# ccaven/tinyslam

Measured on AMD Instinct MI355X. Metric: ORB extract throughput, 1280x720 (frames/sec; Mkeypoints/sec alongside), higher is better.
Workload: dtype f32; 1 GPU; BASELINE.json configs[3]: batch of 256 independent 1280x720 RGBA frames per GPU, device-resident, full ORB (FAST-12 + orientation + blur + BRIEF-256); frames_per_gpu_per_batch=256, width=1280, height=720, hierarchy_depth=2, max_features=8192, content=default, mode=literal, input=rgba, pipeline=default, fp_contract=0, angle_bins=0, batches_in_flight=1, collate=none (1 GPU)

## Files before the change

### include/tinyorb.h

```cpp
#ifndef TINYORB_H
#define TINYORB_H

#include <stddef.h>
#include <stdint.h>

#ifdef __cplusplus
extern "C" {
#endif

#define TINYORB_ABI_VERSION 5

#define ORB_OK 0
#define ORB_EINVAL 1
#define ORB_EHIP 2
#define ORB_ECAPACITY 3
#define ORB_ESTATE 4

#define ORB_MAX_HIERARCHY_DEPTH 10

typedef struct OrbExtent3d {
    uint32_t width;
    uint32_t height;
    uint32_t depth_or_array_layers;
} OrbExtent3d;
// ... 139 lines not shown
    uint32_t reserved[3];
} OrbPairModel;

#define ORB_VERIFY_OK 0u
#define ORB_VERIFY_FEW 1u
#define ORB_VERIFY_DEGENERATE 2u
#define ORB_VERIFY_MINIMAL 3u

int orb_verify_consecutive(OrbProgram *p, uint32_t n_frames, const OrbVerifyParams *params, void *stream);
int orb_verify_read(OrbProgram *p, uint32_t pair, OrbPairModel *model, uint8_t *inlier, size_t n);

void orb_corner_level0_xy(const CornerData *c, float *x0, float *y0);

#define ORB_PLANE_GRAY 0
#define ORB_PLANE_BLUR 1
int orb_debug_read_plane(OrbProgram *p, uint32_t frame, int kind, uint32_t level, uint16_t *dst, size_t n_texels);
int orb_level_size(const OrbProgram *p, uint32_t level, uint32_t *width, uint32_t *height);
int orb_debug_f32_to_f16(OrbProgram *p, const float *src, uint16_t *dst, size_t n);
int orb_debug_angle_code(OrbProgram *p, const float *cy, const float *cx, uint32_t *dst, size_t n);
int orb_debug_rot_table(OrbProgram *p, int16_t *dst, size_t n_entries, uint32_t *codes, uint32_t *pitch);

#define ORB_KERNEL_COUNT 25
int orb_profile_enable(OrbProgram *p, int enable);
int orb_profile_reset(OrbProgram *p);
int orb_profile_get(OrbProgram *p, int id, double *total_ms, uint64_t *launches);
const char *orb_kernel_name(int id);

#define ORB_SYN_GRADIENT 1u
#define ORB_SYN_BLOBS 2u
#define ORB_SYN_WEDGES 4u
// ... 12 lines not shown
```

### tinyslam_amd/csrc/orb_api.hip

```cpp
#include <hip/hip_runtime.h>
#include <chrono>
#include <cmath>

#include <cstdarg>
#include <cstdio>
#include <cstdlib>
#include <cstring>
#include <new>
#include <string>
#include <algorithm>
#include <vector>

#include "../../include/tinyorb.h"
#include "orb_front_launch.h"
#include "orb_kernels_fused.h"
#include "orb_kernels_brief.h"
#include "orb_kernels_intended.h"
#include "orb_kernels_staged.h"
#include "orb_kernels_collate.h"
#include "orb_kernels_match.h"
#include "orb_kernels_verify.h"

using namespace orb;

// ... 110 lines not shown
    uint16_t* d_blur_rowc = nullptr;
    uint32_t blur_qa[kMaxLevels] = {0};
    uint32_t* d_counts = nullptr;
    CornerData* d_corners = nullptr;
    CornerDescriptor* d_desc = nullptr;
    uint32_t* out_counts[2] = {nullptr, nullptr};
    CornerData* out_corners[2] = {nullptr, nullptr};
    CornerDescriptor* out_desc[2] = {nullptr, nullptr};
    CornerData* d_seg = nullptr;
    uint32_t* d_seg_counts = nullptr;
    uint32_t* d_seg_before = nullptr;
    BandGeom bands{};
    RowsGeom rows{};
    BriefTGeom brieft{};
    bool use_brief_t = false;
    uint32_t band_rows_lvl[kMaxLevels] = {0};
    uint32_t ln_threads[kMaxLevels] = {0};
    uint32_t tile_w_lvl[kMaxLevels] = {0};
    uint32_t seg_classes = 1;
    uint32_t* d_pattern = nullptr;
    float* d_cos = nullptr;
    float* d_sin = nullptr;
    uint4* d_rot = nullptr;
    unsigned long long* d_stamps = nullptr;

    uint32_t* h_count = nullptr;
    uint32_t* d_single_done = nullptr;
    hipEvent_t single_done_ev = nullptr;
    uint32_t single_seq = 0;
    CornerData* h_corners = nullptr;
// ... 270 lines not shown
    g.n_classes = n_classes;
    uint32_t rows = 0;
    for (uint32_t m = 0; m < p->pyr.depth; m++) {
        g.flat_end[m] = rg.flat_end[m];
        g.qa[m] = rg.qa[m];
        g.row_base[m] = rows + (uint32_t)kBriefHalo;
        rows += p->pyr.h[m] + 2u * (uint32_t)kBriefHalo + 8u;
    }
    g.rows_padded = rows;
    g.oob = p->oob;
    *out = g;
    if (getenv("TINYORB_BRIEF_ROWS")) return false;
    return rg.n_slots >= 1u && rg.n_slots * n_classes <= kBriefTMaxSlots && rows <= kBriefTMaxRows;
}

int launch_brief(OrbProgram* p, hipStream_t s, uint32_t n, const RowsGeom& rows_geom, const uint16_t* d_blur,
                 const uint16_t* d_blur_rowc, const uint32_t* seg_counts, uint32_t* seg_before, const CornerData* seg,
                 uint32_t* d_counts, CornerData* d_corners, CornerDescriptor* d_desc) {
    const uint32_t cap = p->cfg.max_features;
    const BriefTables tab{p->d_pattern, p->d_cos, p->d_sin, p->d_rot};
    const bool use_t = p->use_brief_t;
    {
        LaunchScope ls(p, s, KID_PREFIX);
        hipLaunchKernelGGL(k_slot_prefix, dim3(n), dim3(64), 0, s, seg_counts, seg_before, d_counts, rows_geom.n_slots,
                           rows_geom.seg_cap, use_t ? p->brieft.n_classes : 1u);
    }
    if (use_t) {
        const BriefTGeom& tg = p->brieft;
        const dim3 grid(n, (cap + (uint32_t)kBriefNfChunk - 1u) / (uint32_t)kBriefNfChunk);
        {
            LaunchScope ls(p, s, KID_BRIEF_T);
#define BRIEF_T_LAUNCH(ROT_)                                                                                                         \
    hipLaunchKernelGGL((k_brief_t<kBriefTWaves, ROT_>), dim3(n, (cap + kBriefTThreads - 1u) / kBriefTThreads), dim3(kBriefTThreads), \
                       brieft_lds_bytes(tg), s, d_blur_rowc, p->pyr, tg, seg_counts, seg_before, seg, d_corners, cap, d_desc, tab)
            switch (rot_form(p->opt.fp_contract)) {
                case 1: BRIEF_T_LAUNCH(1); break;
                case 2: BRIEF_T_LAUNCH(2); break;
                default: BRIEF_T_LAUNCH(0); break;
            }
#undef BRIEF_T_LAUNCH
        }
        LaunchScope ls(p, s, KID_BRIEF_NF);
        if (p->oob != kOobZero)
            hipLaunchKernelGGL(k_brief_nf<true>, grid, dim3(256), 0, s, d_blur, d_blur_rowc, p->pyr, tg, seg_counts, seg_before, d_corners,
                               cap, d_desc, tab);
        else
            hipLaunchKernelGGL(k_brief_nf<false>, grid, dim3(256), 0, s, d_blur, d_blur_rowc, p->pyr, tg, seg_counts, seg_before, d_corners,
                               cap, d_desc, tab);
    } else {
        LaunchScope ls(p, s, KID_BRIEF_ROWS);
        RowsGeom rg = rows_geom;
        rg.oob = p->oob;
        rg.fp = p->opt.fp_contract;
        rg.split = 1u;
        while (rg.split < 16u && rg.n_slots * n * rg.split < 2048u) rg.split *= 2u;
        hipLaunchKernelGGL(k_brief_rows, dim3(rg.n_slots * rg.split, n), dim3(256), 0, s, d_blur, d_blur_rowc, p->pyr, rg,
                           seg_counts, seg_before, seg, d_corners, cap, d_desc, tab);
    }
    return ORB_OK;
}

int run_fused_range(OrbProgram* p, const uint8_t* frames_all, uint32_t f0, uint32_t n, hipStream_t s, bool with_brief = true,
                    uint32_t first_level = 0) {
    const Pyramid& pyr = p->pyr;
// ... 40 lines not shown
        if (!g.tiled && sizeof(BlurCol) * (size_t)g.n_var > 8u * (size_t)g.ts)
            return fail(p, ORB_EINVAL, "internal: blur column table of level %u does not fit", lvl);
        uint32_t lds = front_lds_bytes(g);
        lds += (uint32_t)p->env.lds_pad;
        if (lds > p->max_lds) return fail(p, ORB_EINVAL, "level %u needs %u bytes of LDS", lvl, lds);
        const dim3 grid(g.n_bands * (g.tiled ? g.n_ct : 1u) * n);
        FrontLaunch L{frames, p->frame_bytes, d_gray, d_blur, d_blur_rowc, pyr, g, p->threshold, d_seg_counts, d_seg, s_lvl, grid.x, lds,
                      p->band_rows_lvl[lvl], p->ln_threads[lvl], p->input_y8,
                      lvl == 0 && ((pyr.w[0] & 3u) || g.store_grey), p->oob != kOobZero, false};
        {
            LaunchScope ls(p, s_lvl, lvl == 0 ? KID_FUSED_L0 : KID_FUSED_LN);
            const hipError_t e = kFrontLaunch[front_form(p->opt.fp_contract, lvl == 0 && !p->input_y8)](L);
            if (e != hipSuccess) return fail(p, ORB_EHIP, "k_front (level %u) failed to launch: %s", lvl, hipGetErrorString(e));
        }
    }
    if (with_brief) launch_brief(p, s, n, p->rows, d_blur, d_blur_rowc, d_seg_counts, d_seg_before, d_seg, d_counts, d_corners, d_desc);
    HIP_TRY(p, hipGetLastError());
    return ORB_OK;
}

int run_fused(OrbProgram* p, const uint8_t* frames, uint32_t n, hipStream_t s) {
    if (int rc = run_fused_range(p, frames, 0, n, s)) return rc;
    p->planes_valid = true;
    return ORB_OK;
}

uint32_t itile_width(uint32_t w) {
    const uint32_t w8 = (w + 7u) & ~7u;
    return w8 < (uint32_t)kITileW ? w8 : (uint32_t)kITileW;
}

// ... 146 lines not shown
            fg.slot_base = band_base;
            fg.n_slots = p->xband_slots;
            fg.seg_cap = 1u;
            fg.n_classes = 1u;
            fg.stamps = nullptr;
            band_base += fg.n_bands;
            const uint32_t lds = front_lds_bytes(fg);
            if (lds > p->max_lds) return fail(p, ORB_EINVAL, "level %u needs %u bytes of LDS", lvl, lds);
            LaunchScope ls(p, s, KID_FUSED_LN);
            const FrontLaunch L{frames, p->frame_bytes, p->d_gray, p->d_blur, p->d_blur_rowc, pyr, fg, p->threshold, p->d_xband_counts, p->d_iseg, s,
                                fg.n_bands * n, lds, (uint32_t)kFrontRows, (uint32_t)kFrontThreadsLN, false, false, false, true};
            const hipError_t e = kFrontLaunch[0](L);
            if (e != hipSuccess) return fail(p, ORB_EHIP, "k_front (blur of level %u) failed to launch: %s", lvl, hipGetErrorString(e));
        }
    }
    launch_brief(p, s, n, p->xrows, p->d_blur, p->d_blur_rowc, p->d_iseg_counts, p->d_iseg_before, p->d_iseg, p->d_counts,
                 p->d_corners, p->d_desc);
    HIP_TRY(p, hipGetLastError());
    p->planes_valid = true;
    return ORB_OK;
}

int launch_compact(OrbProgram* p, uint32_t n, uint32_t* counts, uint64_t* offsets, CornerData* corners, CornerDescriptor* desc,
                   size_t capacity, void* stream, hipStream_t* used);

int run_pipeline(OrbProgram* p, const uint8_t* frames, uint32_t n, hipStream_t s) {
    if (p->fused_i) return run_fused_i(p, frames, n, s);
    if (p->fused_x) return run_fused_x(p, frames, n, s);
    return p->fused ? run_fused(p, frames, n, s) : run_staged(p, frames, n, s);
}

// ... 339 lines not shown
    p->d_desc = p->out_desc[0];
    if (p->fused) {
        CREATE_TRY(hipMalloc(&p->d_blur_rowc, B * p->pyr.row_stride * sizeof(uint16_t)));
        CREATE_TRY(hipMemset(p->d_blur_rowc, 0, B * p->pyr.row_stride * sizeof(uint16_t)));
        const size_t lists = (size_t)p->bands.n_slots * p->seg_classes;
        CREATE_TRY(hipMalloc(&p->d_seg, B * lists * (size_t)p->bands.seg_cap * sizeof(CornerData)));
        CREATE_TRY(hipMalloc(&p->d_seg_counts, B * lists * sizeof(uint32_t)));
        CREATE_TRY(hipMemset(p->d_seg_counts, 0, B * lists * sizeof(uint32_t)));
        CREATE_TRY(hipMalloc(&p->d_seg_before, B * lists * sizeof(uint32_t)));
    }
    if (p->fused_x) {
        CREATE_TRY(hipMalloc(&p->d_blur_rowc, B * p->pyr.row_stride * sizeof(uint16_t)));
        CREATE_TRY(hipMemset(p->d_blur_rowc, 0, B * p->pyr.row_stride * sizeof(uint16_t)));
        CREATE_TRY(hipMalloc(&p->d_xband_counts, B * (size_t)p->xband_slots * sizeof(uint32_t)));
    }
    if (p->fused_i || p->fused_x) {
        const size_t n_seg = B * (size_t)p->itiles.n_slots;
        CREATE_TRY(hipMalloc(&p->d_iseg, n_seg * p->itiles.seg_cap * sizeof(CornerData)));
        CREATE_TRY(hipMalloc(&p->d_iseg_scores, n_seg * p->itiles.seg_cap * sizeof(float)));
        CREATE_TRY(hipMalloc(&p->d_iseg_counts, n_seg * sizeof(uint32_t)));
        CREATE_TRY(hipMemset(p->d_iseg_counts, 0, n_seg * sizeof(uint32_t)));
        CREATE_TRY(hipMalloc(&p->d_iseg_before, n_seg * sizeof(uint32_t)));
        CREATE_TRY(hipMalloc(&p->d_thr_key, B * sizeof(unsigned long long)));
    } else if (p->opt.flags & (ORB_FLAG_NMS | ORB_FLAG_INTENDED)) {
        uint32_t off = 0, width = W, height = H;
        for (uint32_t m = 0; m < p->pyr.depth; m++) {
            const uint32_t gw = ((width + 7u) / 8u) * 8u, gh = ((height + 7u) / 8u) * 8u;
            p->score_layout.off[m] = off;
            p->score_layout.pitch[m] = gw + 2u;
            off += (gw + 2u) * (gh + 2u);
// ... 66 lines not shown
    (void)hipFree(p->d_input);
    (void)hipFree(p->d_input_alt);
    for (hipEvent_t ev : p->in_uploaded)
        if (ev) (void)hipEventDestroy(ev);
    (void)hipFree(p->d_gray);
    (void)hipFree(p->d_blur);
    (void)hipFree(p->d_blur_rowc);
    for (int set = 0; set < 2; set++) {
        (void)hipFree(p->out_counts[set]);
        (void)hipFree(p->out_corners[set]);
        (void)hipFree(p->out_desc[set]);
    }
    (void)hipFree(p->d_seg);
    (void)hipFree(p->d_seg_counts);
    (void)hipFree(p->d_seg_before);
    (void)hipFree(p->d_score_planes);
    (void)hipFree(p->d_prov_counts);
    (void)hipFree(p->d_prov);
    (void)hipFree(p->d_prov_scores);
    (void)hipFree(p->d_matches);
    (void)hipFree(p->d_xband_counts);
    (void)hipFree(p->d_iseg);
    (void)hipFree(p->d_iseg_scores);
    (void)hipFree(p->d_iseg_counts);
    (void)hipFree(p->d_iseg_before);
    (void)hipFree(p->d_thr_key);
    (void)hipFree(p->d_prov2_counts);
    (void)hipFree(p->d_prov2);
    (void)hipFree(p->d_prov2_scores);
    (void)hipFree(p->d_pattern);
// ... 767 lines not shown
    if (counts) *counts = p->d_counts;
    if (corners) *corners = p->d_corners;
    if (descriptors) *descriptors = p->d_desc;
    return ORB_OK;
}

int orb_level_size(const OrbProgram* p, uint32_t level, uint32_t* width, uint32_t* height) {
    if (!p || level >= p->pyr.depth) return ORB_EINVAL;
    if (width) *width = p->pyr.w[level];
    if (height) *height = p->pyr.h[level];
    return ORB_OK;
}

int orb_debug_read_plane(OrbProgram* p, uint32_t frame, int kind, uint32_t level, uint16_t* dst, size_t n_texels) {
    if (!p) return ORB_EINVAL;
    if (!dst || level >= p->pyr.depth || frame >= p->last_batch || (kind != ORB_PLANE_GRAY && kind != ORB_PLANE_BLUR))
        return fail(p, ORB_EINVAL, "debug_read_plane: bad arguments");
    if (!p->planes_valid || ((p->fused || (p->fused_i && !p->igrey_stored)) && kind == ORB_PLANE_GRAY && level == 0))
        return fail(p, ORB_ESTATE, "plane not materialised by the last call");
    const size_t texels = (size_t)p->pyr.w[level] * p->pyr.h[level];
    if (n_texels != texels) return fail(p, ORB_EINVAL, "debug_read_plane: expected %zu texels", texels);
    if (int rc = orb_batch_sync(p)) return rc;
    const uint16_t* base = (kind == ORB_PLANE_GRAY ? p->d_gray : p->d_blur) + (size_t)frame * p->pyr.stride + p->pyr.off[level];
    HIP_TRY(p, hipMemcpy(dst, base, texels * sizeof(uint16_t), hipMemcpyDeviceToHost));
    if ((p->fused || p->fused_x) && kind == ORB_PLANE_BLUR && p->blur_qa[level] > 0) {
        const uint32_t w = p->pyr.w[level], h = p->pyr.h[level], qa = p->blur_qa[level];
        std::vector<uint16_t> rowc(h);
        HIP_TRY(p, hipMemcpy(rowc.data(), p->d_blur_rowc + (size_t)frame * p->pyr.row_stride + p->pyr.row_off[level],
                             h * sizeof(uint16_t), hipMemcpyDeviceToHost));
        for (uint32_t y = 0; y < h; y++)
// ... 133 lines not shown
```

### tinyslam_amd/csrc/orb_kernels_brief.h

```cpp
#pragma once
#include "orb_kernels_fused.h"

namespace orb {

constexpr int kBriefTThreads = 256;
constexpr int kBriefTWaves = 6;
constexpr uint32_t kBriefTMaxSlots = 8192;
constexpr uint32_t kBriefTMaxRows = 12288;

struct BriefTGeom {
    uint32_t n_slots, seg_cap;
    uint32_t n_classes;
    uint32_t flat_end[kMaxLevels];
    uint32_t qa[kMaxLevels];
    uint32_t row_base[kMaxLevels];
    uint32_t rows_padded;
    uint32_t oob;
};

__host__ __device__ inline uint32_t brieft_lds_bytes(const BriefTGeom& g) {
    return (g.n_slots * g.n_classes + 1u) * 4u + ((g.rows_padded + 1u) & ~1u) * 2u;
}

__device__ __forceinline__ constexpr int pat_ax(int j) { return ORB_BRIEF_PATTERN[4 * j + 0]; }
// ... 20 lines not shown
}

__device__ __forceinline__ void brief_t_stage_rows(uint16_t* rows, const uint16_t* __restrict__ src, const Pyramid& pyr,
                                                   const BriefTGeom& bg, uint32_t tid, uint32_t n_threads = kBriefTThreads) {
    uint32_t m = 0;
    for (uint32_t i = tid; i < bg.rows_padded; i += n_threads) {
        while (m + 1u < pyr.depth && i + (uint32_t)kBriefHalo >= bg.row_base[m + 1u]) m++;
        const uint32_t y = i - bg.row_base[m];
        uint16_t v = 0;
        if (y < pyr.h[m]) v = src[pyr.row_off[m] + y];
        else if (bg.oob != kOobZero) v = src[pyr.row_off[m] + (uint32_t)oob_index((int)y, (int)pyr.h[m], bg.oob)];
        rows[i] = v;
    }
}

template <int CHUNK = kBriefTThreads, bool STAGED = false, int ROT = 0>
__device__ __forceinline__ void brief_t_body(uint8_t* lds_raw, uint32_t frame, uint32_t chunk, const uint16_t* __restrict__ blur_rowc,
                                             const Pyramid& pyr, const BriefTGeom& bg, const uint32_t* __restrict__ seg_counts,
                                             const uint32_t* __restrict__ seg_before, const CornerData* __restrict__ segments,
                                             CornerData* __restrict__ corners, uint32_t cap,
                                             CornerDescriptor* __restrict__ descriptors, const BriefTables& tab,
                                             CornerData* __restrict__ host_corners = nullptr,
                                             CornerDescriptor* __restrict__ host_descriptors = nullptr) {
    const uint32_t n_ent = bg.n_slots * bg.n_classes;
    uint32_t* const before = reinterpret_cast<uint32_t*>(lds_raw);
    uint16_t* const rows = reinterpret_cast<uint16_t*>(before + n_ent + 1u);
    __shared__ uint32_t lv[kMaxLevels][2];

    const uint32_t tid = threadIdx.x;
    const size_t sbase = (size_t)frame * n_ent;
    uint32_t stored_total;
    if (STAGED) {
        if (tid < pyr.depth) lv[tid][0] = bg.flat_end[tid], lv[tid][1] = bg.row_base[tid];
        __syncthreads();
        stored_total = before[n_ent];
    } else {
        stored_total = seg_before[sbase + n_ent - 1u] + min(seg_counts[sbase + n_ent - 1u], bg.seg_cap);
    }
    const uint32_t n_frame = min(stored_total, cap);
    const uint32_t k0 = chunk * (uint32_t)CHUNK;
    if (k0 >= n_frame) return;

    if (!STAGED) {
        for (uint32_t s = tid; s < n_ent; s += kBriefTThreads) before[s] = seg_before[sbase + s];
        if (tid == 0) before[n_ent] = stored_total;
        if (tid < pyr.depth) lv[tid][0] = bg.flat_end[tid], lv[tid][1] = bg.row_base[tid];
        brief_t_stage_rows(rows, blur_rowc + (size_t)frame * pyr.row_stride, pyr, bg, tid);
        __syncthreads();
    }

    const uint32_t k = k0 + tid;
    if (tid >= (uint32_t)CHUNK || k >= n_frame) return;
    uint32_t lo = 0, hi = n_ent;
    while (hi - lo > 1u) {
        const uint32_t mid = (lo + hi) >> 1;
        if (before[mid] <= k)
            lo = mid;
        else
            hi = mid;
    }
    const uint32_t cls = lo >= bg.n_slots ? 1u : 0u, slot = lo - cls * bg.n_slots;
    const uint4 rec = *reinterpret_cast<const uint4*>(
        &segments[(((size_t)frame * bg.n_slots + slot) * bg.n_classes + cls) * bg.seg_cap + (k - before[lo])]);
    *reinterpret_cast<uint4*>(&corners[(size_t)frame * cap + k]) = rec;
    if (host_corners) store_host_16(&host_corners[k], rec);
    const uint32_t lvl = min(rec.w, pyr.depth - 1u);
    if (!(rec.x >= (uint32_t)kBriefHalo && rec.x < lv[lvl][0])) return;

    uint32_t d[8];
    uint4* const o = reinterpret_cast<uint4*>(descriptors + (size_t)frame * cap + k);
    if (bg.n_classes == 2u && k0 + (tid & ~63u) + 64u <= before[bg.n_slots]) {
        const uint16_t* base0 = rows + lv[lvl][1] + rec.y - kBriefHalo;
#pragma unroll
        for (int wd = 0; wd < 8; wd++) {
            uint32_t acc = 0;
#pragma unroll
            for (int i = 31; i >= 0; i--) {
                const int j = wd * 32 + i;
                acc = push_gt(acc, base0[pat_ay(j) + kBriefHalo], base0[pat_by(j) + kBriefHalo]);
            }
            d[wd] = acc;
        }
// ... 31 lines not shown
            acc = push_gt(acc, base[(int)ray], base[(int)rby]);
        }
        d[wd] = acc;
    }
    o[0] = make_uint4(d[0], d[1], d[2], d[3]);
    o[1] = make_uint4(d[4], d[5], d[6], d[7]);
    if (host_descriptors) {
        store_host_16(reinterpret_cast<uint4*>(host_descriptors + k), make_uint4(d[0], d[1], d[2], d[3]));
        store_host_16(reinterpret_cast<uint4*>(host_descriptors + k) + 1, make_uint4(d[4], d[5], d[6], d[7]));
    }
}

template <int kWavesPerSimd, int ROT = 0>
__global__ __launch_bounds__(kBriefTThreads, kWavesPerSimd) void k_brief_t(const uint16_t* __restrict__ blur_rowc, Pyramid pyr, BriefTGeom bg,
                                                                const uint32_t* __restrict__ seg_counts,
                                                                const uint32_t* __restrict__ seg_before,
                                                                const CornerData* __restrict__ segments,
                                                                CornerData* __restrict__ corners, uint32_t cap,
                                                                CornerDescriptor* __restrict__ descriptors, BriefTables tab) {
    extern __shared__ __attribute__((aligned(16))) uint8_t lds_raw[];
    brief_t_body<kBriefTThreads, false, ROT>(lds_raw, blockIdx.x, blockIdx.y, blur_rowc, pyr, bg, seg_counts, seg_before, segments, corners, cap, descriptors, tab);
}

constexpr int kNfPatchCols = 48, kNfPatchRows = 2 * kBriefHalo + 1;
constexpr int kNfPatchHalfs = kNfPatchRows * kNfPatchCols;

__global__ __launch_bounds__(64) void k_rot_table(const uint32_t* __restrict__ pattern, const float* __restrict__ cos_tab,
                                                  const float* __restrict__ sin_tab, int pitch, int intended, uint4* __restrict__ out,
                                                  uint32_t fp = 0u, uint32_t angle_bins = 0u) {
    const uint32_t code = angle_bins ? (blockIdx.x * 6284u + 3142u) / angle_bins : blockIdx.x, lane = threadIdx.x;
    const float ct = cos_tab[code], st = sin_tab[code], nst = -st;
    uint32_t w[4];
#pragma unroll
    for (int e = 0; e < 4; e++) {
        const uint32_t pk = pattern[64u * (uint32_t)e + lane];
        const float pax = (float)(int8_t)(pk & 255u), pay = (float)(int8_t)((pk >> 8) & 255u);
// ... 2 lines not shown
        if (intended) {
            const float a0 = ct * pax, a1 = nst * pay, a2 = st * pax, a3 = ct * pay;
            const float b0 = ct * pbx, b1 = nst * pby, b2 = st * pbx, b3 = ct * pby;
            rax = a0 + a1, ray = a2 + a3, rbx = b0 + b1, rby = b2 + b3;
        } else {
            rotate_fp(ct, st, nst, pax, pay, rot_form(fp), &rax, &ray);
            rotate_fp(ct, st, nst, pbx, pby, rot_form(fp), &rbx, &rby);
        }
        const int oa = 2 * ((int)ray * pitch + (int)rax), ob = 2 * ((int)rby * pitch + (int)rbx);
        w[e] = ((uint32_t)oa & 0xffffu) | ((uint32_t)ob << 16);
    }
    out[(size_t)blockIdx.x * 64u + lane] = make_uint4(w[0], w[1], w[2], w[3]);
}
__device__ __forceinline__ int rot_a(uint32_t w) { return (int)(int16_t)(w & 0xffffu); }
__device__ __forceinline__ int rot_b(uint32_t w) { return (int)w >> 16; }

template <int CHUNK = 256, int NW = 4, bool OOB = false>
__device__ __forceinline__ void brief_nf_body(uint32_t frame, uint32_t chunk, uint32_t n_known, const uint16_t* __restrict__ blur,
                                              const uint16_t* __restrict__ blur_rowc, const Pyramid& pyr, const BriefTGeom& bg,
                                              const uint32_t* __restrict__ seg_counts, const uint32_t* __restrict__ seg_before,
                                              const CornerData* __restrict__ corners, uint32_t cap,
                                              CornerDescriptor* __restrict__ descriptors, const BriefTables& tab,
                                              CornerDescriptor* __restrict__ host_descriptors = nullptr) {
    static_assert(CHUNK <= 256 && NW >= 4, "the scan runs on the first four waves");
    __shared__ __attribute__((aligned(16))) uint16_t patches[NW][kNfPatchHalfs];
    __shared__ uint4 recs[256];
    __shared__ uint16_t list[256];
    __shared__ uint32_t wave_n[4];
    __shared__ uint32_t lv[kMaxLevels][6];
    const uint32_t tid = threadIdx.x, lane = tid & 63u, wave = tid >> 6;
// ... 127 lines not shown
                    vb = plane[(size_t)(uint32_t)(__mul24(yb, w) + xb)];
                bal[e] = __ballot(va > vb);
            }
        }
        if (lane < 8u) {
            const uint64_t src = lane < 2u ? bal[0] : (lane < 4u ? bal[1] : (lane < 6u ? bal[2] : bal[3]));
            out_desc[(size_t)idx * 8u + lane] = (uint32_t)(src >> ((lane & 1u) * 32u));
            if (host_descriptors) store_host_u32(reinterpret_cast<uint32_t*>(host_descriptors + k0) + (size_t)idx * 8u + lane, (uint32_t)(src >> ((lane & 1u) * 32u)));
        }
    }
}

constexpr int kBriefNfChunk = 64;
template <bool OOB = false>
__global__ __launch_bounds__(256) void k_brief_nf(const uint16_t* __restrict__ blur, const uint16_t* __restrict__ blur_rowc,
                                                  Pyramid pyr, BriefTGeom bg, const uint32_t* __restrict__ seg_counts,
                                                  const uint32_t* __restrict__ seg_before,
                                                  const CornerData* __restrict__ corners, uint32_t cap,
                                                  CornerDescriptor* __restrict__ descriptors, BriefTables tab) {
    brief_nf_body<kBriefNfChunk, 4, OOB>(blockIdx.x, blockIdx.y, ~0u, blur, blur_rowc, pyr, bg, seg_counts, seg_before, corners, cap, descriptors, tab);
}

constexpr int kBriefOneChunk = 64;
constexpr int kSingleCountWords = 32, kSingleDoneWord = 16;
constexpr int kBriefOneThreads = 512;
template <int ROT = 0>
__global__ __launch_bounds__(kBriefOneThreads) void k_brief_one(const uint16_t* __restrict__ blur, const uint16_t* __restrict__ blur_rowc, Pyramid pyr,
                                                   BriefTGeom bg, const uint32_t* __restrict__ seg_counts,
                                                   uint32_t* __restrict__ seg_before, const CornerData* __restrict__ segments,
                                                   uint32_t* __restrict__ counts, CornerData* __restrict__ corners, uint32_t cap,
                                                   CornerDescriptor* __restrict__ descriptors, BriefTables tab,
                                                   uint32_t* __restrict__ host_count, CornerData* __restrict__ host_corners,
                                                   CornerDescriptor* __restrict__ host_descriptors, uint32_t* __restrict__ done_count,
                                                   uint32_t seq) {
    extern __shared__ __attribute__((aligned(16))) uint8_t lds_raw[];
// ... 24 lines not shown
            const uint32_t stored = min(raw, bg.seg_cap);
            const uint32_t incl = wave_inclusive_sum(stored);
            if (e < n_ent) before[e] = carry + incl - stored;
            carry += (uint32_t)__builtin_amdgcn_readlane((int)incl, 63);
            total += (uint32_t)__builtin_amdgcn_readlane((int)wave_inclusive_sum(raw), 63);
        }
        if (tid == 0u) {
            before[n_ent] = carry;
            if (chunk == 0u) {
                counts[0] = total;
                store_host_u32(host_count, total);
            }
        }
    }
    BRIEF_ONE_STAMP();
    brief_t_body<kBriefOneChunk, true, ROT>(lds_raw, 0u, chunk, blur_rowc, pyr, bg, seg_counts, seg_before, segments, corners, cap,
                                       descriptors, tab, host_corners, host_descriptors);
    __syncthreads();
    BRIEF_ONE_STAMP();
    const uint32_t n_stored = before[n_ent];
    brief_nf_body<kBriefOneChunk, kBriefOneThreads / 64>(0u, chunk, n_stored, blur, blur_rowc, pyr, bg, seg_counts, seg_before, corners, cap, descriptors, tab,
                                  host_descriptors);
    BRIEF_ONE_STAMP();
    __builtin_amdgcn_fence(__ATOMIC_RELEASE, "workgroup");
    __builtin_amdgcn_s_waitcnt(0);
    __syncthreads();
    BRIEF_ONE_STAMP();
#ifdef TINYORB_STAMPS
    if (tid == 0u && (chunk == 0u || chunk == 24u))
        for (int i = 0; i < 5; i++) host_count[(chunk ? 6 : 1) + i] = (uint32_t)(st[i + 1] - st[i]);
#endif
// ... 13 lines not shown
```

### tinyslam_amd/orb.py

```python
import ctypes
import importlib.util
import os
from dataclasses import dataclass, field

import numpy as np

_PKG = os.path.dirname(os.path.abspath(__file__))
LIB_PATH = os.environ.get("TINYORB_LIB") or os.path.join(os.path.dirname(os.path.abspath(__file__)), "libtinyorb.so")

ORB_OK, ORB_EINVAL, ORB_EHIP, ORB_ECAPACITY, ORB_ESTATE = 0, 1, 2, 3, 4
ORB_PLANE_GRAY, ORB_PLANE_BLUR = 0, 1
ORB_KERNEL_COUNT = 25
ORB_FLAG_STAGED = 1
ORB_FLAG_DOUBLE_OUTPUT = 2
ORB_FLAG_NMS = 4
ORB_FLAG_INTENDED = 8
ORB_FLAG_INPUT_Y8 = 16
ORB_FLAG_SINGLE_BLOCKING_WAIT = 32
ORB_OOB_ZERO, ORB_OOB_CLAMP, ORB_OOB_UMIN = 0, 1, 2
OOB_POLICIES = {"zero": ORB_OOB_ZERO, "clamp": ORB_OOB_CLAMP, "umin": ORB_OOB_UMIN}
ORB_FP_CONTRACT_LUMINANCE, ORB_FP_CONTRACT_BLUR, ORB_FP_CONTRACT_ROTATION, ORB_FP_CONTRACT_ALL, ORB_FP_LAST_TERM_FIRST = 1, 2, 4, 7, 8
TRANSPORT_RECORD_WORDS = 10
SYN_GRADIENT, SYN_BLOBS, SYN_WEDGES, SYN_NOISE = 1, 2, 4, 8
SYN_ALL = 15

CORNER_DTYPE = np.dtype([("x", "<u4"), ("y", "<u4"), ("angle", "<u4"), ("octave", "<u4")])
# ... 606 lines not shown
```

Baseline: 478,200 frames/s.

## Fold slot prefix into k_brief_t and emit compacted non-flat keypoint lists

Removes the separate k_slot_prefix launch on the k_brief_t path: each brief_t block recomputes the per-frame segment prefix sum in LDS and chunk 0 writes the frame total. brief_t also ballots and compacts keypoints that fall outside the flat fast path into a per-wave list, so k_brief_nf processes only those entries (one wave per keypoint) instead of rescanning all corners. This saves a launch and the nf kernel's scan work, at the cost of redundant prefix work in every block plus extra list memory and writes.

```diff
diff --git a/include/tinyorb.h b/include/tinyorb.h
--- a/include/tinyorb.h
+++ b/include/tinyorb.h
@@ -177,6 +177,7 @@
 
 #define ORB_PLANE_GRAY 0
 #define ORB_PLANE_BLUR 1
+#define ORB_PLANE_NF_COUNT 2
 int orb_debug_read_plane(OrbProgram *p, uint32_t frame, int kind, uint32_t level, uint16_t *dst, size_t n_texels);
 int orb_level_size(const OrbProgram *p, uint32_t level, uint32_t *width, uint32_t *height);
 int orb_debug_f32_to_f16(OrbProgram *p, const float *src, uint16_t *dst, size_t n);
diff --git a/tinyslam_amd/csrc/orb_api.hip b/tinyslam_amd/csrc/orb_api.hip
--- a/tinyslam_amd/csrc/orb_api.hip
+++ b/tinyslam_amd/csrc/orb_api.hip
@@ -148,6 +148,9 @@
     RowsGeom rows{};
     BriefTGeom brieft{};
     bool use_brief_t = false;
+    uint4* d_nf_list = nullptr;
+    uint32_t* d_nf_count = nullptr;
+    uint32_t nf_chunks = 0;
     uint32_t band_rows_lvl[kMaxLevels] = {0};
     uint32_t ln_threads[kMaxLevels] = {0};
     uint32_t tile_w_lvl[kMaxLevels] = {0};
@@ -448,25 +451,20 @@
     return rg.n_slots >= 1u && rg.n_slots * n_classes <= kBriefTMaxSlots && rows <= kBriefTMaxRows;
 }
 
-int launch_brief(OrbProgram* p, hipStream_t s, uint32_t n, const RowsGeom& rows_geom, const uint16_t* d_blur,
+int launch_brief(OrbProgram* p, hipStream_t s, uint32_t f0, uint32_t n, const RowsGeom& rows_geom, const uint16_t* d_blur,
                  const uint16_t* d_blur_rowc, const uint32_t* seg_counts, uint32_t* seg_before, const CornerData* seg,
                  uint32_t* d_counts, CornerData* d_corners, CornerDescriptor* d_desc) {
     const uint32_t cap = p->cfg.max_features;
     const BriefTables tab{p->d_pattern, p->d_cos, p->d_sin, p->d_rot};
-    const bool use_t = p->use_brief_t;
-    {
-        LaunchScope ls(p, s, KID_PREFIX);
-        hipLaunchKernelGGL(k_slot_prefix, dim3(n), dim3(64), 0, s, seg_counts, seg_before, d_counts, rows_geom.n_slots,
-                           rows_geom.seg_cap, use_t ? p->brieft.n_classes : 1u);
-    }
-    if (use_t) {
+    if (p->use_brief_t) {
         const BriefTGeom& tg = p->brieft;
+        const NfList nf{p->d_nf_list + (size_t)f0 * p->nf_chunks * 64u, p->d_nf_count + (size_t)f0 * p->nf_chunks, p->nf_chunks};
         const dim3 grid(n, (cap + (uint32_t)kBriefNfChunk - 1u) / (uint32_t)kBriefNfChunk);
         {
             LaunchScope ls(p, s, KID_BRIEF_T);
 #define BRIEF_T_LAUNCH(ROT_)                                                                                                         \
     hipLaunchKernelGGL((k_brief_t<kBriefTWaves, ROT_>), dim3(n, (cap + kBriefTThreads - 1u) / kBriefTThreads), dim3(kBriefTThreads), \
-                       brieft_lds_bytes(tg), s, d_blur_rowc, p->pyr, tg, seg_counts, seg_before, seg, d_corners, cap, d_desc, tab)
+                       brieft_lds_bytes(tg), s, d_blur_rowc, p->pyr, tg, seg_counts, seg, d_counts, d_corners, cap, d_desc, tab, nf)
             switch (rot_form(p->opt.fp_contract)) {
                 case 1: BRIEF_T_LAUNCH(1); break;
                 case 2: BRIEF_T_LAUNCH(2); break;
@@ -476,12 +474,15 @@
         }
         LaunchScope ls(p, s, KID_BRIEF_NF);
         if (p->oob != kOobZero)
-            hipLaunchKernelGGL(k_brief_nf<true>, grid, dim3(256), 0, s, d_blur, d_blur_rowc, p->pyr, tg, seg_counts, seg_before, d_corners,
-                               cap, d_desc, tab);
+            hipLaunchKernelGGL(k_brief_nf<true>, grid, dim3(256), 0, s, d_blur, d_blur_rowc, p->pyr, tg, nf, cap, d_desc, tab);
         else
-            hipLaunchKernelGGL(k_brief_nf<false>, grid, dim3(256), 0, s, d_blur, d_blur_rowc, p->pyr, tg, seg_counts, seg_before, d_corners,
-                               cap, d_desc, tab);
+            hipLaunchKernelGGL(k_brief_nf<false>, grid, dim3(256), 0, s, d_blur, d_blur_rowc, p->pyr, tg, nf, cap, d_desc, tab);
     } else {
+        {
+            LaunchScope ls(p, s, KID_PREFIX);
+            hipLaunchKernelGGL(k_slot_prefix, dim3(n), dim3(64), 0, s, seg_counts, seg_before, d_counts, rows_geom.n_slots,
+                               rows_geom.seg_cap, 1u);
+        }
         LaunchScope ls(p, s, KID_BRIEF_ROWS);
         RowsGeom rg = rows_geom;
         rg.oob = p->oob;
@@ -552,7 +553,7 @@
             if (e != hipSuccess) return fail(p, ORB_EHIP, "k_front (level %u) failed to launch: %s", lvl, hipGetErrorString(e));
         }
     }
-    if (with_brief) launch_brief(p, s, n, p->rows, d_blur, d_blur_rowc, d_seg_counts, d_seg_before, d_seg, d_counts, d_corners, d_desc);
+    if (with_brief) launch_brief(p, s, f0, n, p->rows, d_blur, d_blur_rowc, d_seg_counts, d_seg_before, d_seg, d_counts, d_corners, d_desc);
     HIP_TRY(p, hipGetLastError());
     return ORB_OK;
 }
@@ -729,7 +730,7 @@
             if (e != hipSuccess) return fail(p, ORB_EHIP, "k_front (blur of level %u) failed to launch: %s", lvl, hipGetErrorString(e));
         }
     }
-    launch_brief(p, s, n, p->xrows, p->d_blur, p->d_blur_rowc, p->d_iseg_counts, p->d_iseg_before, p->d_iseg, p->d_counts,
+    launch_brief(p, s, 0, n, p->xrows, p->d_blur, p->d_blur_rowc, p->d_iseg_counts, p->d_iseg_before, p->d_iseg, p->d_counts,
                  p->d_corners, p->d_desc);
     HIP_TRY(p, hipGetLastError());
     p->planes_valid = true;
@@ -1099,6 +1100,12 @@
         CREATE_TRY(hipMemset(p->d_blur_rowc, 0, B * p->pyr.row_stride * sizeof(uint16_t)));
         CREATE_TRY(hipMalloc(&p->d_xband_counts, B * (size_t)p->xband_slots * sizeof(uint32_t)));
     }
+    if (p->use_brief_t) {
+        p->nf_chunks = 4u * (uint32_t)((cap + kBriefTThreads - 1u) / kBriefTThreads);
+        CREATE_TRY(hipMalloc(&p->d_nf_list, B * p->nf_chunks * 64u * sizeof(uint4)));
+        CREATE_TRY(hipMalloc(&p->d_nf_count, B * p->nf_chunks * sizeof(uint32_t)));
+        CREATE_TRY(hipMemset(p->d_nf_count, 0, B * p->nf_chunks * sizeof(uint32_t)));
+    }
     if (p->fused_i || p->fused_x) {
         const size_t n_seg = B * (size_t)p->itiles.n_slots;
         CREATE_TRY(hipMalloc(&p->d_iseg, n_seg * p->itiles.seg_cap * sizeof(CornerData)));
@@ -1195,6 +1202,8 @@
     (void)hipFree(p->d_seg);
     (void)hipFree(p->d_seg_counts);
     (void)hipFree(p->d_seg_before);
+    (void)hipFree(p->d_nf_list);
+    (void)hipFree(p->d_nf_count);
     (void)hipFree(p->d_score_planes);
     (void)hipFree(p->d_prov_counts);
     (void)hipFree(p->d_prov);
@@ -1992,6 +2001,15 @@
 
 int orb_debug_read_plane(OrbProgram* p, uint32_t frame, int kind, uint32_t level, uint16_t* dst, size_t n_texels) {
     if (!p) return ORB_EINVAL;
+    if (kind == ORB_PLANE_NF_COUNT && dst && level == 0 && frame < p->last_batch) {
+        if (!p->use_brief_t || p->single_valid) return fail(p, ORB_ESTATE, "the last call was no batch of the k_brief_t path");
+        if (n_texels != p->nf_chunks) return fail(p, ORB_EINVAL, "debug_read_plane: expected %u chunk counts", p->nf_chunks);
+        if (int rc = orb_batch_sync(p)) return rc;
+        std::vector<uint32_t> c(p->nf_chunks);
+        HIP_TRY(p, hipMemcpy(c.data(), p->d_nf_count + (size_t)frame * p->nf_chunks, c.size() * sizeof(uint32_t), hipMemcpyDeviceToHost));
+        for (size_t i = 0; i < c.size(); i++) dst[i] = (uint16_t)c[i];
+        return ORB_OK;
+    }
     if (!dst || level >= p->pyr.depth || frame >= p->last_batch || (kind != ORB_PLANE_GRAY && kind != ORB_PLANE_BLUR))
         return fail(p, ORB_EINVAL, "debug_read_plane: bad arguments");
     if (!p->planes_valid || ((p->fused || (p->fused_i && !p->igrey_stored)) && kind == ORB_PLANE_GRAY && level == 0))
diff --git a/tinyslam_amd/csrc/orb_kernels_brief.h b/tinyslam_amd/csrc/orb_kernels_brief.h
--- a/tinyslam_amd/csrc/orb_kernels_brief.h
+++ b/tinyslam_amd/csrc/orb_kernels_brief.h
@@ -58,35 +58,64 @@
     }
 }
 
+struct NfList {
+    uint4* entries;
+    uint32_t* count;
+    uint32_t chunks;
+};
+
 template <int CHUNK = kBriefTThreads, bool STAGED = false, int ROT = 0>
 __device__ __forceinline__ void brief_t_body(uint8_t* lds_raw, uint32_t frame, uint32_t chunk, const uint16_t* __restrict__ blur_rowc,
                                              const Pyramid& pyr, const BriefTGeom& bg, const uint32_t* __restrict__ seg_counts,
-                                             const uint32_t* __restrict__ seg_before, const CornerData* __restrict__ segments,
+                                             const CornerData* __restrict__ segments,
                                              CornerData* __restrict__ corners, uint32_t cap,
                                              CornerDescriptor* __restrict__ descriptors, const BriefTables& tab,
                                              CornerData* __restrict__ host_corners = nullptr,
-                                             CornerDescriptor* __restrict__ host_descriptors = nullptr) {
+                                             CornerDescriptor* __restrict__ host_descriptors = nullptr,
+                                             uint32_t* __restrict__ counts = nullptr, NfList nf = {}) {
     const uint32_t n_ent = bg.n_slots * bg.n_classes;
     uint32_t* const before = reinterpret_cast<uint32_t*>(lds_raw);
     uint16_t* const rows = reinterpret_cast<uint16_t*>(before + n_ent + 1u);
     __shared__ uint32_t lv[kMaxLevels][2];
 
-    const uint32_t tid = threadIdx.x;
-    const size_t sbase = (size_t)frame * n_ent;
+    const uint32_t tid = threadIdx.x, lane = tid & 63u, wave = tid >> 6;
     uint32_t stored_total;
     if (STAGED) {
         if (tid < pyr.depth) lv[tid][0] = bg.flat_end[tid], lv[tid][1] = bg.row_base[tid];
         __syncthreads();
         stored_total = before[n_ent];
     } else {
-        stored_total = seg_before[sbase + n_ent - 1u] + min(seg_counts[sbase + n_ent - 1u], bg.seg_cap);
+        const uint32_t* sc = seg_counts + (size_t)frame * n_ent;
+        uint32_t carry = 0, total = 0;
+        for (uint32_t e0 = 0; e0 < n_ent; e0 += 256u) {
+            uint32_t raw[4];
+#pragma unroll
+            for (int q = 0; q < 4; q++) {
+                const uint32_t e = e0 + 64u * (uint32_t)q + lane;
+                const uint32_t cls = e >= bg.n_slots ? 1u : 0u, sl = e - cls * bg.n_slots;
+                raw[q] = e < n_ent ? sc[sl * bg.n_classes + cls] : 0u;
+            }
+#pragma unroll
+            for (int q = 0; q < 4; q++) {
+                const uint32_t e = e0 + 64u * (uint32_t)q + lane;
+                const uint32_t stored = min(raw[q], bg.seg_cap);
+                const uint32_t incl = wave_inclusive_sum(stored);
+                if ((uint32_t)q == wave && e < n_ent) before[e] = carry + incl - stored;
+                carry += (uint32_t)__builtin_amdgcn_readlane((int)incl, 63);
+                if (chunk == 0u) total += (uint32_t)__builtin_amdgcn_readlane((int)wave_inclusive_sum(raw[q]), 63);
+            }
+        }
+        if (chunk == 0u && tid == 0u) counts[frame] = total;
+        stored_total = carry;
     }
     const uint32_t n_frame = min(stored_total, cap);
     const uint32_t k0 = chunk * (uint32_t)CHUNK;
-    if (k0 >= n_frame) return;
+    if (k0 >= n_frame) {
+        if (!STAGED && tid < 4u) nf.count[(size_t)frame * nf.chunks + 4u * chunk + tid] = 0u;
+        return;
+    }
 
     if (!STAGED) {
-        for (uint32_t s = tid; s < n_ent; s += kBriefTThreads) before[s] = seg_before[sbase + s];
         if (tid == 0) before[n_ent] = stored_total;
         if (tid < pyr.depth) lv[tid][0] = bg.flat_end[tid], lv[tid][1] = bg.row_base[tid];
         brief_t_stage_rows(rows, blur_rowc + (size_t)frame * pyr.row_stride, pyr, bg, tid);
@@ -94,22 +123,34 @@
     }
 
     const uint32_t k = k0 + tid;
-    if (tid >= (uint32_t)CHUNK || k >= n_frame) return;
+    if (STAGED && (tid >= (uint32_t)CHUNK || k >= n_frame)) return;
+    const bool valid = STAGED || k < n_frame;
+    const uint32_t kq = STAGED ? k : min(k, n_frame - 1u);
     uint32_t lo = 0, hi = n_ent;
     while (hi - lo > 1u) {
         const uint32_t mid = (lo + hi) >> 1;
-        if (before[mid] <= k)
+        if (before[mid] <= kq)
             lo = mid;
         else
             hi = mid;
     }
     const uint32_t cls = lo >= bg.n_slots ? 1u : 0u, slot = lo - cls * bg.n_slots;
     const uint4 rec = *reinterpret_cast<const uint4*>(
-        &segments[(((size_t)frame * bg.n_slots + slot) * bg.n_classes + cls) * bg.seg_cap + (k - before[lo])]);
-    *reinterpret_cast<uint4*>(&corners[(size_t)frame * cap + k]) = rec;
+        &segments[(((size_t)frame * bg.n_slots + slot) * bg.n_classes + cls) * bg.seg_cap + (kq - before[lo])]);
+    if (valid) *reinterpret_cast<uint4*>(&corners[(size_t)frame * cap + k]) = rec;
     if (host_corners) store_host_16(&host_corners[k], rec);
     const uint32_t lvl = min(rec.w, pyr.depth - 1u);
-    if (!(rec.x >= (uint32_t)kBriefHalo && rec.x < lv[lvl][0])) return;
+    const bool flat = rec.x >= (uint32_t)kBriefHalo && rec.x < lv[lvl][0];
+    if (!STAGED) {
+        const uint64_t m = __ballot(valid && !flat);
+        const size_t q = (size_t)frame * nf.chunks + 4u * chunk + wave;
+        if (valid && !flat)
+            nf.entries[q * 64u + (uint32_t)__popcll(m & ((1ull << lane) - 1ull))] =
+                make_uint4(rec.x, rec.y, min(rec.z, (uint32_t)(ORB_ANGLE_STEPS - 1)), lvl | (lane << 8));
+        if (lane == 0u) nf.count[q] = (uint32_t)__popcll(m);
+        if (!valid) return;
+    }
+    if (!flat) return;
 
     uint32_t d[8];
     uint4* const o = reinterpret_cast<uint4*>(descriptors + (size_t)frame * cap + k);
@@ -171,12 +212,12 @@
 template <int kWavesPerSimd, int ROT = 0>
 __global__ __launch_bounds__(kBriefTThreads, kWavesPerSimd) void k_brief_t(const uint16_t* __restrict__ blur_rowc, Pyramid pyr, BriefTGeom bg,
                                                                 const uint32_t* __restrict__ seg_counts,
-                                                                const uint32_t* __restrict__ seg_before,
-                                                                const CornerData* __restrict__ segments,
+                                                                const CornerData* __restrict__ segments, uint32_t* __restrict__ counts,
                                                                 CornerData* __restrict__ corners, uint32_t cap,
-                                                                CornerDescriptor* __restrict__ descriptors, BriefTables tab) {
+                                                                CornerDescriptor* __restrict__ descriptors, BriefTables tab, NfList nf) {
     extern __shared__ __attribute__((aligned(16))) uint8_t lds_raw[];
-    brief_t_body<kBriefTThreads, false, ROT>(lds_raw, blockIdx.x, blockIdx.y, blur_rowc, pyr, bg, seg_counts, seg_before, segments, corners, cap, descriptors, tab);
+    brief_t_body<kBriefTThreads, false, ROT>(lds_raw, blockIdx.x, blockIdx.y, blur_rowc, pyr, bg, seg_counts, segments, corners, cap, descriptors,
+                                             tab, nullptr, nullptr, counts, nf);
 }
 
 constexpr int kNfPatchCols = 48, kNfPatchRows = 2 * kBriefHalo + 1;
@@ -209,6 +250,102 @@
 }
 __device__ __forceinline__ int rot_a(uint32_t w) { return (int)(int16_t)(w & 0xffffu); }
 __device__ __forceinline__ int rot_b(uint32_t w) { return (int)w >> 16; }
+
+template <bool OOB>
+__device__ __forceinline__ void brief_nf_key(uint32_t lane, uint16_t* patch, const uint4& r, int w, int h, int qa,
+                                             const uint16_t* __restrict__ rowc, const uint16_t* __restrict__ plane, const BriefTGeom& bg,
+                                             const BriefTables& tab, uint32_t* out_desc, uint32_t idx) {
+    const uint4 tt = tab.rot[(size_t)min(r.z, (uint32_t)(ORB_ANGLE_STEPS - 1)) * 64u + lane];
+    const uint32_t tw[4] = {tt.x, tt.y, tt.z, tt.w};
+    uint64_t bal[4];
+    if ((w & 1) == 0) {
+        const int c0 = ((int)r.x - kBriefHalo) & ~7;
+        constexpr int kPiecesPerRow = kNfPatchCols / 8, kPieces = kNfPatchRows * kPiecesPerRow;
+        constexpr int kRounds = (kPieces + 63) / 64;
+        uint4 tv[kRounds];
+        uint32_t rcv[kRounds];
+        int kind[kRounds], where[kRounds];
+#pragma unroll
+        for (int rr = 0; rr < kRounds; rr++) {
+            const int p = (int)lane + 64 * rr;
+            const int pr = (int)(((float)p + 0.5f) * (1.0f / (float)kPiecesPerRow));
+            const int pc = p - pr * kPiecesPerRow;
+            const int gy0 = (int)r.y - kBriefHalo + pr, cx = c0 + 8 * pc;
+            const int gy = OOB ? oob_index(gy0, h, bg.oob) : gy0;
+            const bool in = p < kPieces && gy >= 0 && gy < h && cx >= 0 && cx < w;
+            kind[rr] = !in ? 0 : (cx < qa ? 1 : (cx + 8 <= w ? 2 : 3));
+            where[rr] = p < kPieces ? pr * kNfPatchCols + 8 * pc : -1;
+            rcv[rr] = rowc[min(max(gy, 0), h - 1)];
+            if (OOB && p < kPieces && !(cx >= 0 && cx < w)) {
+                const int xm = oob_index(cx, w, bg.oob);
+                if (xm >= qa) rcv[rr] = plane[(size_t)(uint32_t)(__mul24(gy, w) + xm)];
+                kind[rr] = 1;
+            }
+            tv[rr] = *reinterpret_cast<const uint4*>(plane + (kind[rr] == 2 ? (size_t)(uint32_t)(__mul24(gy, w) + cx) : (size_t)0));
+        }
+#pragma unroll
+        for (int rr = 0; rr < kRounds; rr++) {
+            uint4 v = make_uint4(0u, 0u, 0u, 0u);
+            if (kind[rr] == 1) {
+                const uint32_t c2 = rcv[rr] | (rcv[rr] << 16);
+                v = make_uint4(c2, c2, c2, c2);
+            } else if (kind[rr] == 2) {
+                v = tv[rr];
+            } else if (kind[rr] == 3) {
+                const int p = (int)lane + 64 * rr;
+                const int pr = (int)(((float)p + 0.5f) * (1.0f / (float)kPiecesPerRow));
+                const int gy0 = (int)r.y - kBriefHalo + pr, cx = c0 + 8 * (p - pr * kPiecesPerRow);
+                const int gy = OOB ? oob_index(gy0, h, bg.oob) : gy0;
+                const uint16_t* src = plane + (size_t)(uint32_t)(__mul24(gy, w) + cx);
+                uint32_t t[8];
+#pragma unroll
+                for (int q = 0; q < 8; q++) t[q] = cx + q < w ? (uint32_t)src[q] : (OOB ? (uint32_t)src[w - 1 - cx] : 0u);
+                v = make_uint4(t[0] | (t[1] << 16), t[2] | (t[3] << 16), t[4] | (t[5] << 16), t[6] | (t[7] << 16));
+            }
+            if (where[rr] >= 0) *reinterpret_cast<uint4*>(&patch[where[rr]]) = v;
+        }
+        __builtin_amdgcn_fence(__ATOMIC_RELEASE, "wavefront");
+        __builtin_amdgcn_wave_barrier();
+        const int xo = (int)r.x - c0;
+        const uint8_t* const centre = reinterpret_cast<const uint8_t*>(patch + kBriefHalo * kNfPatchCols + xo);
+#pragma unroll
+        for (int e = 0; e < 4; e++) {
+            const uint32_t va = *reinterpret_cast<const uint16_t*>(centre + rot_a(tw[e]));
+            const uint32_t vb = *reinterpret_cast<const uint16_t*>(centre + rot_b(tw[e]));
+            bal[e] = __ballot(va > vb);
+        }
+        __builtin_amdgcn_fence(__ATOMIC_RELEASE, "wavefront");
+        __builtin_amdgcn_wave_barrier();
+    } else {
+        const int gy = (int)r.y - kBriefHalo + (int)lane;
+        const uint32_t rowv = (gy >= 0 && gy < h && lane < 37u) ? (uint32_t)rowc[gy] : 0u;
+#pragma unroll
+        for (int e = 0; e < 4; e++) {
+            const int oa = rot_a(tw[e]) >> 1, ob = rot_b(tw[e]) >> 1;
+            const int dya = (oa + kNfPatchCols / 2 + 64 * kNfPatchCols) / kNfPatchCols - 64, dxa = oa - dya * kNfPatchCols;
+            const int dyb = (ob + kNfPatchCols / 2 + 64 * kNfPatchCols) / kNfPatchCols - 64, dxb = ob - dyb * kNfPatchCols;
+            const int xa = (int)r.x + dxa, ya = (int)r.y + dya;
+            const int xb = (int)r.x + dxb, yb = (int)r.y + dyb;
+            uint32_t va = (uint32_t)__shfl((int)rowv, dya + kBriefHalo);
+            uint32_t vb = (uint32_t)__shfl((int)rowv, dyb + kBriefHalo);
+            const bool ina = xa >= 0 && xa < w && ya >= 0 && ya < h;
+            const bool inb = xb >= 0 && xb < w && yb >= 0 && yb < h;
+            if (!ina)
+                va = OOB ? blur_sample_mapped(plane, rowc, w, h, qa, xa, ya, bg.oob) : 0u;
+            else if (xa >= qa)
+                va = plane[(size_t)(uint32_t)(__mul24(ya, w) + xa)];
+            if (!inb)
+                vb = OOB ? blur_sample_mapped(plane, rowc, w, h, qa, xb, yb, bg.oob) : 0u;
+            else if (xb >= qa)
+                vb = plane[(size_t)(uint32_t)(__mul24(yb, w) + xb)];
+            bal[e] = __ballot(va > vb);
+        }
+    }
+    if (lane < 8u) {
+        const uint64_t src = lane < 2u ? bal[0] : (lane < 4u ? bal[1] : (lane < 6u ? bal[2] : bal[3]));
+        out_desc[(size_t)idx * 8u + lane] = (uint32_t)(src >> ((lane & 1u) * 32u));
+    }
+}
 
 template <int CHUNK = 256, int NW = 4, bool OOB = false>
 __device__ __forceinline__ void brief_nf_body(uint32_t frame, uint32_t chunk, uint32_t n_known, const uint16_t* __restrict__ blur,
@@ -366,11 +503,32 @@
 constexpr int kBriefNfChunk = 64;
 template <bool OOB = false>
 __global__ __launch_bounds__(256) void k_brief_nf(const uint16_t* __restrict__ blur, const uint16_t* __restrict__ blur_rowc,
-                                                  Pyramid pyr, BriefTGeom bg, const uint32_t* __restrict__ seg_counts,
-                                                  const uint32_t* __restrict__ seg_before,
-                                                  const CornerData* __restrict__ corners, uint32_t cap,
+                                                  Pyramid pyr, BriefTGeom bg, NfList nf, uint32_t cap,
                                                   CornerDescriptor* __restrict__ descriptors, BriefTables tab) {
-    brief_nf_body<kBriefNfChunk, 4, OOB>(blockIdx.x, blockIdx.y, ~0u, blur, blur_rowc, pyr, bg, seg_counts, seg_before, corners, cap, descriptors, tab);
+    __shared__ __attribute__((aligned(16))) uint16_t patches[4][kNfPatchHalfs];
+    const uint32_t frame = blockIdx.x, chunk = blockIdx.y;
+    const uint32_t lane = threadIdx.x & 63u, wave = __builtin_amdgcn_readfirstlane(threadIdx.x >> 6);
+    const size_t q = (size_t)frame * nf.chunks + chunk;
+    const uint4* const ent = nf.entries + q * 64u;
+    const uint32_t n_nf = nf.count[q];
+    uint4 e = ent[wave];
+    if (wave >= n_nf) return;
+    uint32_t gw = 0, gh = 0, gqa = 0, grow = 0, goff = 0;
+#pragma unroll
+    for (int m = 0; m < kMaxLevels; m++)
+        if (lane == (uint32_t)m) gw = pyr.w[m], gh = pyr.h[m], gqa = bg.qa[m], grow = pyr.row_off[m], goff = pyr.off[m];
+    uint32_t* const out_desc = reinterpret_cast<uint32_t*>(descriptors + (size_t)frame * cap + chunk * (uint32_t)kBriefNfChunk);
+    uint16_t* const patch = patches[wave];
+    for (uint32_t i = wave; i < n_nf; i += 4u) {
+        if (i != wave) e = ent[i];
+        const uint32_t lvl = __builtin_amdgcn_readfirstlane(e.w & 255u), idx = __builtin_amdgcn_readfirstlane(e.w >> 8);
+        const uint4 r = make_uint4(__builtin_amdgcn_readfirstlane(e.x), __builtin_amdgcn_readfirstlane(e.y), __builtin_amdgcn_readfirstlane(e.z), lvl);
+        const int w = __builtin_amdgcn_readlane((int)gw, (int)lvl), h = __builtin_amdgcn_readlane((int)gh, (int)lvl);
+        const int qa = __builtin_amdgcn_readlane((int)gqa, (int)lvl);
+        const uint16_t* rowc = blur_rowc + (size_t)frame * pyr.row_stride + (uint32_t)__builtin_amdgcn_readlane((int)grow, (int)lvl);
+        const uint16_t* plane = blur + (size_t)frame * pyr.stride + (uint32_t)__builtin_amdgcn_readlane((int)goff, (int)lvl);
+        brief_nf_key<OOB>(lane, patch, r, w, h, qa, rowc, plane, bg, tab, out_desc, idx);
+    }
 }
 
 constexpr int kBriefOneChunk = 64;
@@ -425,7 +583,7 @@
         }
     }
     BRIEF_ONE_STAMP();
-    brief_t_body<kBriefOneChunk, true, ROT>(lds_raw, 0u, chunk, blur_rowc, pyr, bg, seg_counts, seg_before, segments, corners, cap,
+    brief_t_body<kBriefOneChunk, true, ROT>(lds_raw, 0u, chunk, blur_rowc, pyr, bg, seg_counts, segments, corners, cap,
                                        descriptors, tab, host_corners, host_descriptors);
     __syncthreads();
     BRIEF_ONE_STAMP();
diff --git a/tinyslam_amd/orb.py b/tinyslam_amd/orb.py
--- a/tinyslam_amd/orb.py
+++ b/tinyslam_amd/orb.py
@@ -9,7 +9,7 @@
 LIB_PATH = os.environ.get("TINYORB_LIB") or os.path.join(os.path.dirname(os.path.abspath(__file__)), "libtinyorb.so")
 
 ORB_OK, ORB_EINVAL, ORB_EHIP, ORB_ECAPACITY, ORB_ESTATE = 0, 1, 2, 3, 4
-ORB_PLANE_GRAY, ORB_PLANE_BLUR = 0, 1
+ORB_PLANE_GRAY, ORB_PLANE_BLUR, ORB_PLANE_NF_COUNT = 0, 1, 2
 ORB_KERNEL_COUNT = 25
 ORB_FLAG_STAGED = 1
 ORB_FLAG_DOUBLE_OUTPUT = 2
```

After: 477,800 frames/s (median of 3 runs). About the same (-0.1%).
